# dropbox/divans

Hardware: AMD Instinct MI355X
Metric: MB/s encode+decode per GPU, 64 KiB metablocks; bit-exact vs CPU (higher is better)
Workload: dtype u16/u64 integer

## Files before the change

### divans_amd/csrc/lit_bucket.hip

```cpp
#include "lit_bucket_dev.h"

#ifndef DIVANS_BK_CHAIN_NO_STORES
#define DIVANS_BK_CHAIN_NO_STORES 0
#endif

namespace divans_hip {

__global__ __launch_bounds__(BK_SORT_THREADS) void bucket_sort_kernel(const BucketBatch b) {
    __shared__ __attribute__((aligned(16))) unsigned long long staging64[BK_PIECE / 8u];
    uint8_t* staging = (uint8_t*)staging64;
    __shared__ __attribute__((aligned(16))) uint8_t piece_in[16 + BK_PIECE];
    __shared__ uint32_t hist[4][256];
    __shared__ uint32_t wsum[4];
    const uint32_t s = blockIdx.x / b.pieces, piece = blockIdx.x % b.pieces;
    const uint32_t tid = threadIdx.x, w = (uint32_t)__builtin_amdgcn_readfirstlane((int)(tid >> 6)), lane = tid & 63;
    const uint32_t len = b.in_sizes ? b.in_sizes[s] : b.stream_len;
    const uint8_t* in = b.in + (b.in_offsets ? b.in_offsets[s] : (uint64_t)s * b.stream_len);
    uint32_t* desc = b.desc + ((size_t)s * 256u + tid) * 8u + piece;
    const uint32_t base = piece * BK_PIECE;
    if (base >= len) { *desc = 0u; return; }
    const uint32_t n = len - base < BK_PIECE ? len - base : BK_PIECE;
    const size_t pl = b.slot;
    for (uint32_t i = tid; i < 1024u; i += BK_SORT_THREADS) (&hist[0][0])[i] = 0u;
    {
        const uint8_t* src = in + base;
        if ((((uintptr_t)src) & 15u) == 0u) {
            for (uint32_t i = tid * 16u; i < n; i += BK_SORT_THREADS * 16u) {
                if (i + 16u <= n) *(u32x4*)(piece_in + 16u + i) = *(const u32x4*)(src + i);
                else for (uint32_t k = i; k < n; ++k) piece_in[16u + k] = src[k];
            }
        } else {
            for (uint32_t i = tid; i < n; i += BK_SORT_THREADS) piece_in[16u + i] = src[i];
        }
        if (tid == 0u) piece_in[15] = base ? in[base - 1u] : 0u;
    }
    __syncthreads();
    const uint8_t* key_of = piece_in + 15;
    unsigned long long* mask_of = staging64 + w * 256u;
    const unsigned long long my_bit = 1ull << lane;
    uint32_t kept[16];
#pragma unroll
    for (uint32_t bt = 0; bt < 32u; ++bt) {
        uint32_t r = 0;
        const uint32_t p = w * 2048u + bt * 64u + lane;
        if (p < n) {
            const uint32_t key = key_of[p];
            __hip_atomic_store(mask_of + key, 0ull, __ATOMIC_RELAXED, __HIP_MEMORY_SCOPE_WORKGROUP);
            __hip_atomic_fetch_or(mask_of + key, my_bit, __ATOMIC_RELAXED, __HIP_MEMORY_SCOPE_WORKGROUP);
            const unsigned long long same = __hip_atomic_load(mask_of + key, __ATOMIC_RELAXED, __HIP_MEMORY_SCOPE_WORKGROUP);
            const uint32_t rank = lanes_below(same), cnt = (uint32_t)__popcll(same);
            const uint32_t before = hist[w][key];
            r = before + rank;
            if (rank == cnt - 1u) hist[w][key] = before + cnt;
        }
        if (bt & 1u) kept[bt >> 1] |= r << 16; else kept[bt >> 1] = r;
    }
    __syncthreads();
    const uint32_t c0 = hist[0][tid], c1 = hist[1][tid], c2 = hist[2][tid], c3 = hist[3][tid];
    const uint32_t tot = c0 + c1 + c2 + c3;
    uint32_t incl = tot;
    for (uint32_t d = 1; d < 64u; d <<= 1) {
        const uint32_t v = (uint32_t)__shfl_up((int)incl, d, 64);
        if (lane >= d) incl += v;
    }
    if (lane == 63u) wsum[w] = incl;
    __syncthreads();
    uint32_t start = incl - tot;
    for (uint32_t j = 0; j < 3u; ++j) if (j < w) start += wsum[j];
    hist[0][tid] = start; hist[1][tid] = start + c0; hist[2][tid] = start + c0 + c1; hist[3][tid] = start + c0 + c1 + c2;
    *desc = start | (tot << 16);
    __syncthreads();
    uint16_t* inv = b.inv + (size_t)s * pl + base;
#pragma unroll
    for (uint32_t bt = 0; bt < 32u; ++bt) {
        const uint32_t p = w * 2048u + bt * 64u + lane;
        if (p < n) {
            const uint32_t key = key_of[p], byte = key_of[p + 1u];
            const uint32_t slot = hist[w][key] + ((kept[bt >> 1] >> (16u * (bt & 1u))) & 0xffffu);
            staging[slot] = (uint8_t)byte;
            inv[p] = (uint16_t)slot;
        }
    }
    __syncthreads();
    uint8_t* sorted = b.sorted + (size_t)s * pl + base;
    for (uint32_t i = tid * 16u; i < n; i += BK_SORT_THREADS * 16u) {
        if (i + 16u <= n) *(u32x4*)(sorted + i) = *(const u32x4*)(staging + i);
        else for (uint32_t k = i; k < n; ++k) sorted[k] = staging[k];
    }
}

__global__ __launch_bounds__(1024) void bucket_tasks_kernel(const BucketBatch b) {
    __shared__ uint32_t cnt[BK_CLASSES], basev[BK_CLASSES];
    const uint32_t t = blockIdx.x * 1024u + threadIdx.x;
    const uint32_t cap = b.n_streams * 256u;
    if (threadIdx.x < BK_CLASSES) cnt[threadIdx.x] = 0u;
    __syncthreads();
    uint32_t tot = 0;
    if (t < cap) {
        const u32x4* d = (const u32x4*)(b.desc + (size_t)t * 8u);
        const u32x4 d0 = d[0], d1 = d[1];
        tot = (d0.x >> 16) + (d0.y >> 16) + (d0.z >> 16) + (d0.w >> 16) + (d1.x >> 16) + (d1.y >> 16) + (d1.z >> 16) + (d1.w >> 16);
    }
    const int cls = bk_class_of(tot);
    uint32_t local = 0;
    for (int c = 0; c < (int)BK_CLASSES; ++c) {
        const unsigned long long m = __ballot(cls == c);
        if (m == 0ull) continue;
        const int leader = __ffsll((long long)m) - 1;
        uint32_t wbase = 0;
        if ((int)(threadIdx.x & 63u) == leader) wbase = atomicAdd(&cnt[c], (uint32_t)__popcll(m));
        wbase = (uint32_t)__builtin_amdgcn_readlane((int)wbase, leader);
        if (cls == c) local = wbase + lanes_below(m);
    }
    __syncthreads();
    if (threadIdx.x < BK_CLASSES) basev[threadIdx.x] = cnt[threadIdx.x] ? atomicAdd(&b.counters[threadIdx.x], cnt[threadIdx.x]) : 0u;
    __syncthreads();
    if (cls >= 0) b.tasks[(size_t)cls * cap + basev[cls] + local] = t;
}

__global__ __launch_bounds__(64) void bucket_chain_kernel(const BucketBatch b) {
    extern __shared__ __attribute__((aligned(16))) uint32_t lds32[];
    const uint32_t lane = threadIdx.x;
    uint32_t* my = lds32 + lane * BK_LANE_DWORDS;
    uint32_t* mydesc = my + BK_DESC_DW;
    uint32_t* tab = lds32 + BK_TAB_DW;
    const uint32_t inc = (uint32_t)b.inc; const int lim = b.lim;
    for (uint32_t i = lane; i < 128u; i += 64u) {
        tab[i] = bk_tab_entry(i, inc);
    }
    __syncthreads();
    const size_t pl = b.slot;
    const uint32_t cap = b.n_streams * 256u;
    BkTaskLists lists; lists.load(b.counters);
    const uint32_t total = lists.total();
    const u32x4 def0 = {4u | (8u << 16), 12u | (16u << 16), 20u | (24u << 16), 28u | (32u << 16)};
    const u32x4 def1 = {36u | (40u << 16), 44u | (48u << 16), 52u | (56u << 16), 60u | (64u << 16)};

    bool has_task = false, exhausted = false;
    uint32_t run_i = 0, nruns = 0, left = 0, idx = 0;
    u32x2* cur_sfs = b.sfs; const uint8_t* cur_sorted = b.sorted;
    uint32_t nt_stage = 0, nt_tid = 0;
    u32x4 nd0 = {0u, 0u, 0u, 0u}, nd1 = {0u, 0u, 0u, 0u};
    uint32_t win_cur = 0, win_end = 0, nxt_val = 0, nxt_w = 0;
    const uint32_t long_end = lists.ends[3];
    bool nxt_pending = false, drained = false;
    u32x2 e_next = {0u, 0u}; uint32_t m_next = 0;
    u32x2 pv0 = {0u, 0u}, pv1 = pv0, pv2 = pv0, pv3 = pv0, pv4 = pv0, pv5 = pv0, pv6 = pv0, pv7 = pv0;
    uint32_t m_prev = 0; u32x2* sfs_prev = b.sfs;

#define BK_OPAQUE(X) asm volatile("" : "+v"(X))
#define BK_BYTE(K, WORD, PV)                                                                            \
    if (((K - first) & 15u) < cnt) {                                                                    \
        const uint32_t byte_ = (WORD >> (8u * (K & 3u))) & 0xffu;                                       \
        const uint32_t hi = byte_ >> 4, lo = byte_ & 15u;                                               \
        uint32_t* rowl = my + 8u * (1u + hi);                                                           \
        BkRow H = bk_read(my, tab, hi), L = bk_read(rowl, tab, lo);                                     \
        const u32x2 v = {bk_pack(H, hi), bk_pack(L, lo)};                                               \
        bk_add(H); bk_add(L);                                                                           \
        bk_renorm_at(H, lim); bk_renorm_at(L, lim);                                                     \
        *(u32x4*)my = H.w0; *(u32x4*)(my + 4) = H.w1; *(u32x4*)rowl = L.w0; *(u32x4*)(rowl + 4) = L.w1; \
        PV = v;                                                                                         \
    }

    for (;;) {
        u32x2 e = e_next; const uint32_t m = m_next;
#if DIVANS_BK_CHAIN_NO_STORES
        asm volatile("" : : "v"(pv0), "v"(pv1), "v"(pv2), "v"(pv3), "v"(pv4), "v"(pv5), "v"(pv6), "v"(pv7), "v"(sfs_prev));
        if (false) {
#else
        if (m_prev & BK_VALID) {
#endif
            u32x2* dst = sfs_prev + (m_prev & 0xffffu);
            const uint32_t pf = (m_prev >> 16) & 15u, pc = (m_prev >> 20) & 15u;
            if (pc == 8u) {
                const u32x4 q0 = {pv0.x, pv0.y, pv1.x, pv1.y}, q1 = {pv2.x, pv2.y, pv3.x, pv3.y};
                const u32x4 q2 = {pv4.x, pv4.y, pv5.x, pv5.y}, q3 = {pv6.x, pv6.y, pv7.x, pv7.y};
                bk_store_quad((u32x4*)dst, q0); bk_store_quad((u32x4*)(dst + 2), q1);
                bk_store_quad((u32x4*)(dst + 4), q2); bk_store_quad((u32x4*)(dst + 6), q3);
            } else {
                if (((0u - pf) & 15u) < pc) bk_store_pair(dst + 0, pv0);
                if (((1u - pf) & 15u) < pc) bk_store_pair(dst + 1, pv1);
                if (((2u - pf) & 15u) < pc) bk_store_pair(dst + 2, pv2);
                if (((3u - pf) & 15u) < pc) bk_store_pair(dst + 3, pv3);
                if (((4u - pf) & 15u) < pc) bk_store_pair(dst + 4, pv4);
                if (((5u - pf) & 15u) < pc) bk_store_pair(dst + 5, pv5);
                if (((6u - pf) & 15u) < pc) bk_store_pair(dst + 6, pv6);
                if (((7u - pf) & 15u) < pc) bk_store_pair(dst + 7, pv7);
            }
        }
        {
            const bool adv = has_task && left == 0u, more = run_i < nruns;
            const uint32_t d = mydesc[run_i & 7u];
            if (adv && more) { left = d >> 16; idx = d & 0xffffu; ++run_i; }
            if (adv && !more) has_task = false;
        }
        {
            const bool fetch_ = has_task && left != 0u;
            const uint32_t base = idx & ~7u, first_ = idx & 7u;
            const uint32_t cnt_ = left < 8u - first_ ? left : 8u - first_;
            const uint8_t* lp = fetch_ ? cur_sorted + base : b.sorted;
            e_next = *(const u32x2*)lp;
            m_next = fetch_ ? (base | (first_ << 16) | (cnt_ << 20) | BK_VALID) : 0u;
            idx += fetch_ ? cnt_ : 0u; left -= fetch_ ? cnt_ : 0u;
        }
        BK_OPAQUE(e);
        m_prev = m; sfs_prev = cur_sfs;
        if (m & BK_VALID) {
            const uint32_t first = (m >> 16) & 15u, cnt = (m >> 20) & 15u;
            BK_BYTE(0u, e.x, pv0) BK_BYTE(1u, e.x, pv1) BK_BYTE(2u, e.x, pv2) BK_BYTE(3u, e.x, pv3)
            BK_BYTE(4u, e.y, pv4) BK_BYTE(5u, e.y, pv5) BK_BYTE(6u, e.y, pv6) BK_BYTE(7u, e.y, pv7)
        }
        if (!has_task && !(m_next & BK_VALID) && nt_stage == 3u) {
            BK_OPAQUE(nd0); BK_OPAQUE(nd1);
            uint32_t n = 0;
            const uint32_t dsc[8] = {nd0.x, nd0.y, nd0.z, nd0.w, nd1.x, nd1.y, nd1.z, nd1.w};
#pragma unroll
            for (uint32_t j = 0; j < 8u; ++j) if (dsc[j] >> 16) { mydesc[n] = dsc[j] + j * BK_PIECE; ++n; }
            nruns = n; run_i = 0u;
            for (uint32_t r = 0; r < 17u; ++r) { *(u32x4*)(my + 8u * r) = def0; *(u32x4*)(my + 8u * r + 4u) = def1; }
            cur_sfs = b.sfs + (size_t)(nt_tid >> 8) * pl; cur_sorted = b.sorted + (size_t)(nt_tid >> 8) * pl;
            left = 0u; has_task = true; nt_stage = 0u;
        }
        const bool want = nt_stage == 0u && !exhausted;
        if (nt_stage == 2u) nt_stage = 3u;
        else if (nt_stage == 1u) {
            BK_OPAQUE(nt_tid);
            const u32x4* dp = (const u32x4*)(b.desc + (size_t)nt_tid * 8u);
            nd0 = dp[0]; nd1 = dp[1];
            nt_stage = 2u;
        }
        const unsigned long long wm = __ballot(want);
        if (wm) {
            if (win_cur == win_end && nxt_pending) {
                BK_OPAQUE(nxt_val);
                const uint32_t basev = (uint32_t)__builtin_amdgcn_readfirstlane((int)nxt_val);
                nxt_pending = false;
                if (basev >= total) { drained = true; win_cur = win_end = total; }
                else { win_cur = basev; win_end = basev + nxt_w < total ? basev + nxt_w : total; }
            }
            const uint32_t avail = win_end - win_cur, asked = (uint32_t)__popcll(wm);
            const uint32_t rank = lanes_below(wm);
            if (want) {
                if (rank < avail) {
                    const uint32_t t = win_cur + rank;
                    nt_tid = *lists.at(b.tasks, cap, t);
                    nt_stage = 1u;
                } else if (drained) exhausted = true;
            }
            win_cur += asked < avail ? asked : avail;
        }
        const uint32_t want_w = win_end < long_end ? 64u : BK_WINDOW;
        if (!nxt_pending && !drained && win_end - win_cur < want_w / 2u) {
            nxt_w = want_w;
            if (lane == 0u) nxt_val = atomicAdd(&b.counters[BK_CLAIM], want_w);
            nxt_pending = true;
        }
        const bool done = !has_task && !(m_next & BK_VALID) && !(m_prev & BK_VALID) && nt_stage == 0u && exhausted;
        if (__ballot(!done) == 0ull) break;
    }
#undef BK_BYTE
#undef BK_OPAQUE
}

__global__ __launch_bounds__(1024) void bucket_unsort_kernel(const BucketBatch b) {
    __shared__ u32x2 buf[BK_PIECE];
    const uint32_t s = blockIdx.x / b.pieces, piece = blockIdx.x % b.pieces;
    const uint32_t len = b.in_sizes ? b.in_sizes[s] : b.stream_len;
    const uint32_t base = piece * BK_PIECE;
    if (base >= len) return;
    const uint32_t n = len - base < BK_PIECE ? len - base : BK_PIECE;
    const size_t pl = b.slot;
    const u32x2* src = b.sfs + (size_t)s * pl + base;
    for (uint32_t i = threadIdx.x; i < n; i += 1024u) buf[i] = __builtin_nontemporal_load(src + i);
    __syncthreads();
    const uint16_t* inv = b.inv + (size_t)s * pl + base;
    u32x2* dst = (u32x2*)(b.sf + (size_t)s * b.sf_stride) + base;
    for (uint32_t i = threadIdx.x; i < n; i += 1024u) dst[i] = buf[inv[i]];
}

__global__ __launch_bounds__(1024) void bucket_unsort32_kernel(const BucketBatch b) {
    __shared__ uint32_t buf[BK_PIECE];
    const uint32_t s = blockIdx.x / b.pieces, piece = blockIdx.x % b.pieces;
    const uint32_t len = b.in_sizes ? b.in_sizes[s] : b.stream_len;
    const uint32_t base = piece * BK_PIECE;
    if (base >= len) return;
    const uint32_t n = len - base < BK_PIECE ? len - base : BK_PIECE;
    const size_t pl = b.slot;
    const uint32_t* src = (const uint32_t*)b.sfs + (size_t)s * pl + base;
    const uint32_t n2 = (n + 1u) & ~1u;
    for (uint32_t i = 2u * threadIdx.x; i < n2; i += 2048u) *(u32x2*)(buf + i) = __builtin_nontemporal_load((const u32x2*)(src + i));
    __syncthreads();
    const uint16_t* inv = b.inv + (size_t)s * pl + base;
    uint32_t* dst = b.sf + (size_t)s * b.sf_stride + base;
    for (uint32_t i = 2u * threadIdx.x; i < n2; i += 2048u) {
        const uint32_t iv = *(const uint32_t*)(inv + i);
        const u32x2 v = {buf[iv & 0xffffu], i + 1u < n ? buf[iv >> 16] : 0u};
        *(u32x2*)(dst + i) = v;
    }
}

uint32_t bucket_chain_lds_bytes() { return (64u * BK_LANE_DWORDS + 128u) * 4u; }

void launch_bucket_tasks(const BucketBatch& b, hipStream_t st) {
    hipLaunchKernelGGL(bucket_tasks_kernel, dim3((b.n_streams + 3u) / 4u), dim3(1024), 0, st, b);
}
void launch_bucket_unsort(const BucketBatch& b, hipStream_t st) {
    hipLaunchKernelGGL(bucket_unsort_kernel, dim3(b.n_streams * b.pieces), dim3(1024), 0, st, b);
}

void launch_bucket_unsort32(const BucketBatch& b, hipStream_t st) {
    hipLaunchKernelGGL(bucket_unsort32_kernel, dim3(b.n_streams * b.pieces), dim3(1024), 0, st, b);
}

hipError_t launch_bucket_model(const BucketBatch& b, uint32_t chain_blocks, hipStream_t st) {
    hipError_t e = hipMemsetAsync(b.counters, 0, 64, st);
    if (e != hipSuccess) return e;
    if (b.pieces < 8u) {
        e = hipMemsetAsync(b.desc, 0, (size_t)b.n_streams * 256u * 8u * sizeof(uint32_t), st);
        if (e != hipSuccess) return e;
    }
    hipLaunchKernelGGL(bucket_sort_kernel, dim3(b.n_streams * b.pieces), dim3(BK_SORT_THREADS), 0, st, b);
    hipLaunchKernelGGL(bucket_tasks_kernel, dim3((b.n_streams + 3u) / 4u), dim3(1024), 0, st, b);
#if DIVANS_BK_CHAIN_NO_STORES
    e = hipMemsetD32Async((hipDeviceptr_t)b.sfs, (int)(1u | (2048u << 16)), (size_t)b.n_streams * b.slot * 2u, st);
    if (e != hipSuccess) return e;
#endif
    hipLaunchKernelGGL(bucket_chain_kernel, dim3(chain_blocks), dim3(64), bucket_chain_lds_bytes(), st, b);
    hipLaunchKernelGGL(bucket_unsort_kernel, dim3(b.n_streams * b.pieces), dim3(1024), 0, st, b);
    return hipGetLastError();
}

}
```

### divans_amd/csrc/lit_bucket_dev.h

```cpp
#ifndef DIVANS_LIT_BUCKET_DEV_H_
#define DIVANS_LIT_BUCKET_DEV_H_
#include "lit_device.h"

namespace divans_hip {

constexpr uint32_t BK_PIECE = 8192;
constexpr uint32_t BK_SORT_THREADS = 256;
constexpr uint32_t BK_LANE_DWORDS = 148;
constexpr uint32_t BK_DESC_DW = 136;
constexpr uint32_t BK_TAB_DW = 64 * BK_LANE_DWORDS;
constexpr uint32_t BK_VALID = 1u << 31;
constexpr uint32_t BK_WINDOW = 256;
constexpr uint32_t BK_CLASSES = 6;
constexpr uint32_t BK_CLAIM = 8;

__device__ __forceinline__ int bk_class_of(uint32_t tot) {
    return tot == 0u ? -1 : (tot >= 16384u ? 0 : (tot >= 8192u ? 1 : (tot >= 4096u ? 2 : (tot >= 2048u ? 3 : (tot >= 64u ? 4 : 5)))));
}
struct BkTaskLists {
    uint32_t ends[BK_CLASSES];
    __device__ __forceinline__ void load(const uint32_t* counters) {
        uint32_t acc = 0;
#pragma unroll
        for (uint32_t c = 0; c < BK_CLASSES; ++c) { acc += counters[c]; ends[c] = acc; }
    }
    __device__ __forceinline__ uint32_t total() const { return ends[BK_CLASSES - 1u]; }
    __device__ __forceinline__ const uint32_t* at(const uint32_t* tasks, uint32_t cap, uint32_t t) const {
        uint32_t cls = 0, base = 0;
#pragma unroll
        for (uint32_t c = 0; c + 1u < BK_CLASSES; ++c) if (t >= ends[c]) { cls = c + 1u; base = ends[c]; }
        return tasks + (size_t)cls * cap + (t - base);
    }
};

__device__ __forceinline__ uint32_t lanes_below(unsigned long long m) {
    return __builtin_amdgcn_mbcnt_hi((uint32_t)(m >> 32), __builtin_amdgcn_mbcnt_lo((uint32_t)m, 0u));
}

struct BkRow { u32x4 w0, w1, a0, a1; int chi, cprev; };

__device__ __forceinline__ BkRow bk_read(const uint32_t* row, const uint32_t* tab, uint32_t sym) {
    BkRow r;
    r.w0 = *(const u32x4*)row; r.w1 = *(const u32x4*)(row + 4);
    const uint16_t* r16 = (const uint16_t*)row;
    r.chi = r16[sym];
    r.cprev = r16[sym ? sym - 1u : 0u];
    r.a0 = *(const u32x4*)(tab + sym * 8u); r.a1 = *(const u32x4*)(tab + sym * 8u + 4u);
    return r;
}
__device__ __forceinline__ uint32_t bk_pack(const BkRow& r, uint32_t sym) {
    const int mx = (int)(r.w1.w >> 16);
    const int clo = sym ? r.cprev : 0;
    const float rcp = biased_rcp15(mx);
    const uint32_t dhi = scaled_div(r.chi, mx, rcp), dlo = scaled_div(clo, mx, rcp);
    return (dlo + 1u) | ((dhi - dlo - 1u) << 16);
}
__device__ __forceinline__ void bk_renorm(BkRow& r) {
    const u32x4 b0 = {1u | (2u << 16), 3u | (4u << 16), 5u | (6u << 16), 7u | (8u << 16)};
    const u32x4 b1 = {9u | (10u << 16), 11u | (12u << 16), 13u | (14u << 16), 15u | (16u << 16)};
    const u32x4 t0 = r.w0 + b0, t1 = r.w1 + b1;
    r.w0 = t0 - ((t0 >> 2) & 0x3fff3fffu);
    r.w1 = t1 - ((t1 >> 2) & 0x3fff3fffu);
}

__device__ __forceinline__ uint32_t bk_tab_entry(uint32_t i, uint32_t inc) {
    const uint32_t sym = i >> 3, k = i & 7u;
    return (2u * k >= sym ? inc : 0u) | (2u * k + 1u >= sym ? inc << 16 : 0u);
}
__device__ __forceinline__ void bk_add(BkRow& r) { r.w0 += r.a0; r.w1 += r.a1; }
__device__ __forceinline__ void bk_renorm_at(BkRow& r, int lim) { if ((int)(r.w1.w >> 16) >= lim) bk_renorm(r); }

__device__ __forceinline__ void bk_store_quad(u32x4* p, u32x4 v) {
    asm volatile("global_store_dwordx4 %0, %1, off" : : "v"(p), "v"(v) : "memory");
}
__device__ __forceinline__ void bk_store_pair(u32x2* p, u32x2 v) {
    asm volatile("global_store_dwordx2 %0, %1, off" : : "v"(p), "v"(v) : "memory");
}
__device__ __forceinline__ void bk_store_word(uint32_t* p, uint32_t v) {
    asm volatile("global_store_dword %0, %1, off" : : "v"(p), "v"(v) : "memory");
}

}
#endif
```

Baseline: 15090.

## Software-pipeline LDS row and increment loads across bytes in bucket chain

Splits the per-byte row read into separate row and increment-table requests. The row for byte K+1 and the increments for byte K+2 are issued while byte K's update and pack are still in flight, rotating between two pairs of BkRow registers. Scheduling barriers and opaque asm pin the ordering, so LDS latency overlaps the division math instead of sitting on the serial chain. Renormalization is also rewritten to use packed 16-bit vector arithmetic instead of masked 32-bit shifts. The cost is higher register pressure and speculative LDS reads for bytes that may be invalid.

```diff
diff --git a/divans_amd/csrc/lit_bucket.hip b/divans_amd/csrc/lit_bucket.hip
--- a/divans_amd/csrc/lit_bucket.hip
+++ b/divans_amd/csrc/lit_bucket.hip
@@ -149,17 +149,36 @@
     uint32_t m_prev = 0; u32x2* sfs_prev = b.sfs;
 
 #define BK_OPAQUE(X) asm volatile("" : "+v"(X))
-#define BK_BYTE(K, WORD, PV)                                                                            \
+    uint32_t rd_dw = lane * BK_LANE_DWORDS; BK_OPAQUE(rd_dw);
+    const uint32_t* my_rd = lds32 + rd_dw;
+#define BK_PIN() do { asm volatile("" ::: "memory"); __builtin_amdgcn_sched_barrier(0); } while (0)
+#define BK_VALUE(K) (((K < 4u ? e.x : e.y) >> (8u * (K & 3u))) & 0xffu)
+#define BK_REQUEST_INC(K, H, L) { const uint32_t b_ = BK_VALUE(K); bk_request_inc(H, tab, b_ >> 4); bk_request_inc(L, tab, b_ & 15u); }
+#define BK_REQUEST_ROWS(K, H, L)                                                                        \
+    {                                                                                                   \
+        const uint32_t b_ = BK_VALUE(K);                                                                \
+        bk_request_row(H, my_rd, b_ >> 4); bk_request_row(L, my_rd + 8u * (1u + (b_ >> 4)), b_ & 15u);  \
+    }
+#define BK_UPDATE(K, H, L)                                                                              \
     if (((K - first) & 15u) < cnt) {                                                                    \
-        const uint32_t byte_ = (WORD >> (8u * (K & 3u))) & 0xffu;                                       \
-        const uint32_t hi = byte_ >> 4, lo = byte_ & 15u;                                               \
-        uint32_t* rowl = my + 8u * (1u + hi);                                                           \
-        BkRow H = bk_read(my, tab, hi), L = bk_read(rowl, tab, lo);                                     \
-        const u32x2 v = {bk_pack(H, hi), bk_pack(L, lo)};                                               \
+        uint32_t* rowl = my + 8u * (1u + (BK_VALUE(K) >> 4));                                           \
         bk_add(H); bk_add(L);                                                                           \
         bk_renorm_at(H, lim); bk_renorm_at(L, lim);                                                     \
         *(u32x4*)my = H.w0; *(u32x4*)(my + 4) = H.w1; *(u32x4*)rowl = L.w0; *(u32x4*)(rowl + 4) = L.w1; \
-        PV = v;                                                                                         \
+    }
+#define BK_BYTE(K, H, L, Hn, Ln, PV)                                                                    \
+    {                                                                                                   \
+        const uint32_t byte_ = BK_VALUE(K), hi = byte_ >> 4, lo = byte_ & 15u;                          \
+        int mxh = (int)(H.w1.w >> 16), mxl = (int)(L.w1.w >> 16);             \
+        BK_UPDATE(K, H, L)                                                                              \
+        if (K < 7u) BK_REQUEST_ROWS(K + 1u, Hn, Ln)                                                     \
+        if (K < 6u) BK_REQUEST_INC(K + 2u, H, L)                                                        \
+        BK_PIN();                                                                                       \
+        BK_OPAQUE(mxh); BK_OPAQUE(mxl);                                                                 \
+        u32x2 v = {bk_pack_of(H.chi, H.cprev, mxh, hi), bk_pack_of(L.chi, L.cprev, mxl, lo)};           \
+        BK_OPAQUE(v);                                                                                   \
+        BK_PIN();                                                                                       \
+        if (((K - first) & 15u) < cnt) PV = v;                                                          \
     }
 
     for (;;) {
@@ -207,8 +226,11 @@
         m_prev = m; sfs_prev = cur_sfs;
         if (m & BK_VALID) {
             const uint32_t first = (m >> 16) & 15u, cnt = (m >> 20) & 15u;
-            BK_BYTE(0u, e.x, pv0) BK_BYTE(1u, e.x, pv1) BK_BYTE(2u, e.x, pv2) BK_BYTE(3u, e.x, pv3)
-            BK_BYTE(4u, e.y, pv4) BK_BYTE(5u, e.y, pv5) BK_BYTE(6u, e.y, pv6) BK_BYTE(7u, e.y, pv7)
+            BkRow A, B, C, D;
+            BK_REQUEST_INC(0u, A, B) BK_REQUEST_ROWS(0u, A, B) BK_REQUEST_INC(1u, C, D)
+            BK_PIN();
+            BK_BYTE(0u, A, B, C, D, pv0) BK_BYTE(1u, C, D, A, B, pv1) BK_BYTE(2u, A, B, C, D, pv2) BK_BYTE(3u, C, D, A, B, pv3)
+            BK_BYTE(4u, A, B, C, D, pv4) BK_BYTE(5u, C, D, A, B, pv5) BK_BYTE(6u, A, B, C, D, pv6) BK_BYTE(7u, C, D, A, B, pv7)
         }
         if (!has_task && !(m_next & BK_VALID) && nt_stage == 3u) {
             BK_OPAQUE(nd0); BK_OPAQUE(nd1);
@@ -259,6 +281,11 @@
         if (__ballot(!done) == 0ull) break;
     }
 #undef BK_BYTE
+#undef BK_UPDATE
+#undef BK_REQUEST_ROWS
+#undef BK_REQUEST_INC
+#undef BK_VALUE
+#undef BK_PIN
 #undef BK_OPAQUE
 }
 
diff --git a/divans_amd/csrc/lit_bucket_dev.h b/divans_amd/csrc/lit_bucket_dev.h
--- a/divans_amd/csrc/lit_bucket_dev.h
+++ b/divans_amd/csrc/lit_bucket_dev.h
@@ -39,28 +39,38 @@
 
 struct BkRow { u32x4 w0, w1, a0, a1; int chi, cprev; };
 
-__device__ __forceinline__ BkRow bk_read(const uint32_t* row, const uint32_t* tab, uint32_t sym) {
-    BkRow r;
+__device__ __forceinline__ void bk_request_row(BkRow& r, const uint32_t* row, uint32_t sym) {
     r.w0 = *(const u32x4*)row; r.w1 = *(const u32x4*)(row + 4);
     const uint16_t* r16 = (const uint16_t*)row;
     r.chi = r16[sym];
     r.cprev = r16[sym ? sym - 1u : 0u];
+}
+__device__ __forceinline__ void bk_request_inc(BkRow& r, const uint32_t* tab, uint32_t sym) {
     r.a0 = *(const u32x4*)(tab + sym * 8u); r.a1 = *(const u32x4*)(tab + sym * 8u + 4u);
+}
+__device__ __forceinline__ BkRow bk_read(const uint32_t* row, const uint32_t* tab, uint32_t sym) {
+    BkRow r;
+    bk_request_row(r, row, sym);
+    bk_request_inc(r, tab, sym);
     return r;
 }
-__device__ __forceinline__ uint32_t bk_pack(const BkRow& r, uint32_t sym) {
-    const int mx = (int)(r.w1.w >> 16);
-    const int clo = sym ? r.cprev : 0;
+__device__ __forceinline__ uint32_t bk_pack_of(int chi, int cprev, int mx, uint32_t sym) {
+    const int clo = sym ? cprev : 0;
     const float rcp = biased_rcp15(mx);
-    const uint32_t dhi = scaled_div(r.chi, mx, rcp), dlo = scaled_div(clo, mx, rcp);
+    const uint32_t dhi = scaled_div(chi, mx, rcp), dlo = scaled_div(clo, mx, rcp);
     return (dlo + 1u) | ((dhi - dlo - 1u) << 16);
 }
+__device__ __forceinline__ uint32_t bk_pack(const BkRow& r, uint32_t sym) { return bk_pack_of(r.chi, r.cprev, (int)(r.w1.w >> 16), sym); }
+typedef uint16_t u16x2 __attribute__((ext_vector_type(2)));
+__device__ __forceinline__ uint32_t bk_renorm_dword(uint32_t w, uint32_t bias) {
+    const u16x2 t = __builtin_bit_cast(u16x2, w) + __builtin_bit_cast(u16x2, bias);
+    return __builtin_bit_cast(uint32_t, (u16x2)(t - (t >> 2)));
+}
 __device__ __forceinline__ void bk_renorm(BkRow& r) {
-    const u32x4 b0 = {1u | (2u << 16), 3u | (4u << 16), 5u | (6u << 16), 7u | (8u << 16)};
-    const u32x4 b1 = {9u | (10u << 16), 11u | (12u << 16), 13u | (14u << 16), 15u | (16u << 16)};
-    const u32x4 t0 = r.w0 + b0, t1 = r.w1 + b1;
-    r.w0 = t0 - ((t0 >> 2) & 0x3fff3fffu);
-    r.w1 = t1 - ((t1 >> 2) & 0x3fff3fffu);
+    r.w0.x = bk_renorm_dword(r.w0.x, 1u | (2u << 16)); r.w0.y = bk_renorm_dword(r.w0.y, 3u | (4u << 16));
+    r.w0.z = bk_renorm_dword(r.w0.z, 5u | (6u << 16)); r.w0.w = bk_renorm_dword(r.w0.w, 7u | (8u << 16));
+    r.w1.x = bk_renorm_dword(r.w1.x, 9u | (10u << 16)); r.w1.y = bk_renorm_dword(r.w1.y, 11u | (12u << 16));
+    r.w1.z = bk_renorm_dword(r.w1.z, 13u | (14u << 16)); r.w1.w = bk_renorm_dword(r.w1.w, 15u | (16u << 16));
 }
 
 __device__ __forceinline__ uint32_t bk_tab_entry(uint32_t i, uint32_t inc) {
```

After: 15080. Within noise of the previous version (-0.0%).
